# xyyandhtl/IsaacgymLoco

Measured on AMD Instinct MI355X. Metric: env-steps/sec (whole node), higher is better.
Workload: dtype f32; 1 GPU; aliengo: HIMOnPolicyRunner loop, 9 whole PPO iteration(s) timed, each = 100 x (policy inference + LeggedRobot.step + storage) + GAE + HIMPPO.update (5 epochs x 4 minibatches), 4096 envs/GPU; task=aliengo, envs_per_gpu=4096, mode=train, parallelism=dp1, mixed_robots=False, full=False

## Files before the change

### include/lsim.h

```cpp
#ifndef LSIM_H
#define LSIM_H

#include <stddef.h>
#include <stdint.h>

#ifdef __cplusplus
extern "C" {
#endif

#define LSIM_ABI_VERSION 7

#define LSIM_NUM_DOF 12
#define LSIM_NUM_BODIES 17
#define LSIM_NUM_LEGS 4
#define LSIM_NUM_ACTIONS 12
#define LSIM_ONE_STEP_OBS 45
#define LSIM_OBS_HISTORY 6
#define LSIM_NUM_OBS 270
#define LSIM_MAX_HEIGHT_PTS_X 32
#define LSIM_MAX_HEIGHT_PTS_Y 32
#define LSIM_NUM_HEIGHT_PTS 187
#define LSIM_NUM_PRIV_OBS 238
#define LSIM_NUM_AMP_OBS 30
#define LSIM_NUM_BASE_HEIGHT_PTS 63
// ... 374 lines not shown

int lsim_policy_act_at(const lsim_him_policy* p, const lsim_rollout_storage* st, int64_t step_idx, int64_t draw_counter,
                       const float* obs, const float* priv_obs, const float* std, uint32_t seed, uint32_t rank,
                       float* mean_out, float* values_out, float* actions_out, void* stream);

int lsim_policy_act_post_at(const lsim_him_policy* p, const lsim_rollout_storage* st, int64_t step_idx, int64_t draw_counter,
                            const float* obs, const float* priv_obs, const float* std, uint32_t seed, uint32_t rank,
                            float* mean_out, float* values_out, float* actions_out,
                            int64_t prev_step, const uint8_t* prev_dones, const uint8_t* prev_time_outs, const float* prev_rewards,
                            const float* prev_term_priv_obs, float gamma, void* stream);

typedef struct lsim_policy_extra {
    const float* rows;
    int32_t dim, ld;
    float* store;
} lsim_policy_extra;
int lsim_policy_forward_ext(const lsim_him_policy* p, const lsim_policy_extra* extra, const float* obs, const float* priv_obs, int64_t num_envs,
                            float* mean_out, float* values_out, void* stream);
int lsim_policy_act_post_at_ext(const lsim_him_policy* p, const lsim_policy_extra* extra, const lsim_rollout_storage* st, int64_t step_idx,
                                int64_t draw_counter, const float* obs, const float* priv_obs, const float* std, uint32_t seed, uint32_t rank,
                                float* mean_out, float* values_out, float* actions_out,
                                int64_t prev_step, const uint8_t* prev_dones, const uint8_t* prev_time_outs, const float* prev_rewards,
                                const float* prev_term_priv_obs, float gamma, void* stream);

typedef struct lsim_amp_disc {
    lsim_mlp_layer hidden[2];
    const float* head_weight;
    const float* head_bias;
    const double* norm_mean;
    const double* norm_var;
    double norm_eps, norm_clip;
    double reward_coef, task_reward_lerp;
    int32_t amp_dim, reserved;
} lsim_amp_disc;
int lsim_amp_step_workspace(int64_t num_envs, size_t* bytes);
int lsim_amp_step(const lsim_amp_disc* d, const float* amp_obs, const float* next_amp_obs, const uint8_t* dones, const float* terminal_amp_states,
                  const float* task_rewards, int64_t num_envs, float* rewards_out, float* disc_out, float* amp_obs_carry,
                  float* replay_states, float* replay_next_states, int64_t replay_capacity, int64_t replay_cursor,
                  void* workspace, size_t workspace_bytes, void* stream);

int lsim_linear_wgrad_workspace(long batch, int k_in, int n_out, size_t* bytes, int* num_waves);
int lsim_linear_wgrad(const float* x, int64_t ldx, const float* g, int64_t ldg, int64_t batch, int k_in, int n_out,
                      float* dw, float* db, void* workspace, size_t workspace_bytes, void* stream);

int lsim_linear_elu_forward(const float* x, int64_t ldx, const float* weight, const float* bias, int64_t batch, int k_in, int n_out,
                            float* out, int64_t ldo, void* stream);

int lsim_linear_elu_wgrad(const float* x, int64_t ldx, const float* grad_out, int64_t ldg, const float* elu_out, int64_t ldz, int64_t batch,
                          int k_in, int n_out, float* dw, float* db, float* grad_pre, void* workspace, size_t workspace_bytes, void* stream);

int lsim_linear_relu_wgrad(const float* x, int64_t ldx, const float* grad_out, int64_t ldg, const float* relu_out, int64_t ldz, int64_t batch,
                           int k_in, int n_out, float* dw, float* db, float* grad_pre, void* workspace, size_t workspace_bytes, void* stream);

int lsim_linear_masked_forward(const float* x, int64_t ldx, const float* weight, const float* mask_src, int64_t ldm, int64_t batch, int k_in, int n_out,
                               float* out, int64_t ldo, void* stream);

int lsim_relu_cols_workspace(int64_t batch, int n, size_t* bytes);
int lsim_relu_head_backward(const float* relu_out, int64_t ld, const float* grad_d, const float* head_weight, int64_t batch, int n,
                            float* grad_pre, float* grad_bias, float* grad_head, void* workspace, size_t workspace_bytes, void* stream);
int lsim_masked_colsum(const float* v, int64_t ldv, const float* mask_src, int64_t ldm, int64_t batch, int n, float* out,
                       void* workspace, size_t workspace_bytes, void* stream);

int lsim_running_moments_workspace(size_t* bytes);
int lsim_running_moments_update(const float* x, int64_t ldx, int64_t batch, int dim, double* mean, double* var, double* count,
                                void* workspace, size_t workspace_bytes, void* stream);

int lsim_amp_pair_rows(const float* states, int64_t ld_states, const float* next_states, int64_t ld_next, const double* norm_mean,
                       const double* norm_var, double norm_eps, double norm_clip, int64_t batch, int dim, float* out, int64_t ld_out, void* stream);

typedef struct lsim_wgrad_pending {
    const float* part; const float* part2;
    float* out; float* out2;
    int32_t num_partials, count, count2, reserved;
} lsim_wgrad_pending;
int lsim_linear_wgrad_deferred(const float* x, int64_t ldx, const float* g, int64_t ldg, int64_t batch, int k_in, int n_out,
                               float* dw, float* db, void* workspace, size_t workspace_bytes, void* stream, lsim_wgrad_pending* pending);
int lsim_linear_elu_wgrad_deferred(const float* x, int64_t ldx, const float* grad_out, int64_t ldg, const float* elu_out, int64_t ldz, int64_t batch,
                                   int k_in, int n_out, float* dw, float* db, float* grad_pre, void* workspace, size_t workspace_bytes, void* stream,
                                   lsim_wgrad_pending* pending);
int lsim_linear_relu_wgrad_deferred(const float* x, int64_t ldx, const float* grad_out, int64_t ldg, const float* relu_out, int64_t ldz, int64_t batch,
                                    int k_in, int n_out, float* dw, float* db, float* grad_pre, void* workspace, size_t workspace_bytes, void* stream,
                                    lsim_wgrad_pending* pending);
int lsim_wgrad_reduce_batch(const lsim_wgrad_pending* items, int n, void* stream);

int lsim_gather_rows(const void* src, int64_t cols, const int64_t* index, int64_t n, void* dst, void* stream);
int lsim_gather_rows_ld(const void* src, int64_t cols, const int64_t* index, int64_t n, void* dst, int64_t dst_ld, void* stream);

int lsim_normalize_rows(float* w, int rows, int cols, float eps, void* stream);

int lsim_ppo_loss_workspace(long batch, size_t* bytes);
int lsim_ppo_loss(const float* mu, const float* sigma, const float* value, const float* actions, const float* old_logp, const float* advantages,
                  const float* returns, const float* target_values, const float* old_mu, const float* old_sigma, int64_t batch, int num_actions,
                  float clip_param, float value_loss_coef, float entropy_coef, int use_clipped_value_loss,
                  float* out5, float* grad_mu, float* grad_sigma, float* grad_value, void* workspace, size_t workspace_bytes, void* stream);
int lsim_ppo_loss_std_workspace(long batch, int num_actions, size_t* bytes);
int lsim_ppo_loss_std(const float* mu, const float* std, const float* value, const float* actions, const float* old_logp, const float* advantages,
                      const float* returns, const float* target_values, const float* old_mu, const float* old_sigma, int64_t batch, int num_actions,
                      float clip_param, float value_loss_coef, float entropy_coef, int use_clipped_value_loss,
                      float* out5, float* grad_mu, float* grad_std, float* grad_value, void* workspace, size_t workspace_bytes, void* stream);


int lsim_adaptive_lr(const float* kl_mean_dev, float desired_kl, float lr_min, float lr_max, float factor, float* lr_dev, void* stream);

int lsim_sinkhorn_workspace(long batch, int K, size_t* bytes);
int lsim_sinkhorn(const float* scores, int64_t lds, int64_t batch, int K, float eps, int iters, float* out,
                  void* workspace, size_t workspace_bytes, void* stream);

int lsim_estimator_loss_workspace(int64_t batch, int latent, int K, size_t* bytes);
int lsim_estimator_loss(const float* enc_out, int64_t ld_enc, const float* tgt_out, int64_t ld_tgt, const float* proto, const float* vel,
                        int64_t ld_vel, int64_t batch, int latent, int K, float temperature, float sinkhorn_eps, int sinkhorn_iters,
                        float* losses3, float* grad_enc, float* grad_tgt, float* grad_proto, void* workspace, size_t workspace_bytes,
                        void* stream);

int lsim_adam_clip_step_workspace(int count, size_t* bytes);
int lsim_adam_clip_step(int count, const int64_t* numel, float* const* params, float* const* grads, float* const* exp_avg,
                        float* const* exp_avg_sq, float* const* steps, const float* lr_dev, float lr_host, float beta1, float beta2,
                        float eps, float max_grad_norm, float* grad_norm_out, void* workspace, size_t workspace_bytes, void* stream);

int lsim_adam_clip_step_ex(int count, const int64_t* numel, float* const* params, float* const* grads, float* const* exp_avg,
                           float* const* exp_avg_sq, float* const* steps, const float* weight_decay, int clip_count,
                           const float* lr_dev, float lr_host, float beta1, float beta2, float eps, float max_grad_norm,
                           float* grad_norm_out, void* workspace, size_t workspace_bytes, void* stream);

int lsim_actor_input(const float* obs, int64_t ld_obs, int num_one_step_obs, const float* enc_out, int64_t ld_enc, int latent,
                     int64_t batch, float* out, void* stream);

#define LSIM_EVAL_BY_ROBOT 1u
#define LSIM_EVAL_BY_TYPE 2u
#define LSIM_EVAL_BY_LEVEL 4u
#define LSIM_EVAL_MAX_GROUPS 4096
#define LSIM_EVAL_MAX_TRACE_ENVS 64
#define LSIM_EVAL_SAT_PERMILLE 980
enum lsim_eval_word {
    LSIM_EVAL_W_SAMPLES = 0,
    LSIM_EVAL_W_LIN_ERR,
    LSIM_EVAL_W_LIN_ERR_SQ,
    LSIM_EVAL_W_YAW_ERR,
    LSIM_EVAL_W_YAW_ERR_SQ,
    LSIM_EVAL_W_POWER,
    LSIM_EVAL_W_TORQUE_SQ,
    LSIM_EVAL_W_ACTION_RATE,
    LSIM_EVAL_W_FEET_CONTACT,
    LSIM_EVAL_W_TORQUE_SAT,
    LSIM_EVAL_W_PEAK_TORQUE_RATIO,
    LSIM_EVAL_W_EPISODES,
    LSIM_EVAL_W_TIME_OUTS,
    LSIM_EVAL_W_FALLS,
    LSIM_EVAL_W_RETURN,
    LSIM_EVAL_W_LENGTH,
    LSIM_EVAL_W_DISTANCE,
    LSIM_EVAL_W_NONFINITE,
    LSIM_EVAL_WORDS
};
#define LSIM_EVAL_TR_DOF_POS_TARGET 0
#define LSIM_EVAL_TR_DOF_POS 12
#define LSIM_EVAL_TR_DOF_VEL 24
#define LSIM_EVAL_TR_TORQUES 36
#define LSIM_EVAL_TR_COMMANDS 48
#define LSIM_EVAL_TR_BASE_LIN_VEL 51
#define LSIM_EVAL_TR_BASE_ANG_VEL 54
#define LSIM_EVAL_TR_CONTACT_FORCES_Z 57
#define LSIM_EVAL_TR_ROOT_POS 61
#define LSIM_EVAL_TR_ROOT_QUAT 64
#define LSIM_EVAL_TR_REW 68
#define LSIM_EVAL_TR_RESET 69
#define LSIM_EVAL_TRACE_DIM 70
// ... 431 lines not shown
```

### isaacgymloco_amd/csrc/ls_learn.h

```cpp
#pragma once
#include <hip/hip_runtime.h>

typedef float ls_v4f __attribute__((ext_vector_type(4)));

#define LS_WGRAD_WAVES_PER_BLOCK 4

template <int NT, int KT>
__global__ __launch_bounds__(64 * LS_WGRAD_WAVES_PER_BLOCK) void lsim_k_linear_wgrad(const float* __restrict__ x, long ldx, const float* __restrict__ g, long ldg,
                                                                                    long batch, int k_in, int n_out, long rows_per_wave,
                                                                                    float* __restrict__ part_dw, float* __restrict__ part_db) {
    const int lane = threadIdx.x & 63, wave = blockIdx.x * LS_WGRAD_WAVES_PER_BLOCK + (threadIdx.x >> 6);
    const int sub = lane >> 4, col = lane & 15;
    const long b0 = (long)wave * rows_per_wave;
    if (b0 >= batch) return;
    long b1 = b0 + rows_per_wave;
    if (b1 > batch) b1 = batch;
    ls_v4f acc[NT][KT];
    float dbacc[NT];
#pragma unroll
    for (int nt = 0; nt < NT; ++nt) {
        dbacc[nt] = 0.0f;
#pragma unroll
        for (int kt = 0; kt < KT; ++kt) acc[nt][kt] = (ls_v4f){0.0f, 0.0f, 0.0f, 0.0f};
    }
// ... 518 lines not shown
        }
        if (bad) return LSIM_E_UNSUPPORTED;
    } else {
        const int tiles = p.n_blocks * p.k_blocks;
        const int blocks = tiles * p.partials;
        const int vx = ((ldx % 4 == 0) && (((uintptr_t)x & 15) == 0)) ? 2 : (((ldx % 2 == 0) && (((uintptr_t)x & 7) == 0)) ? 1 : 0);
        int vg = ((ldg % 4 == 0) && (((uintptr_t)g & 15) == 0)) ? 2 : 0;
        if (fz && !((ldz % 4 == 0) && (((uintptr_t)z & 15) == 0))) vg = 0;
        const int kg = k_in <= 64 ? 1 : 2;
#define LS_T(VX, VG, KG, FZ) hipLaunchKernelGGL((lsim_k_linear_wgrad_tiled<VX, VG, KG, FZ>), dim3(blocks), dim3(256), 0, s, x, (long)ldx, g, (long)ldg, z, (long)ldz, \
                                                gy, (long)batch, k_in, n_out, p.k_blocks, tiles, p.partials, p.rows, pdw, pdb, zoff)
#define LS_TZ(VX, VG, KG) do { if (fz) LS_T(VX, VG, KG, true); else LS_T(VX, VG, KG, false); } while (0)
#define LS_TK(VX, VG) do { if (kg == 1) LS_TZ(VX, VG, 1); else LS_TZ(VX, VG, 2); } while (0)
        if (vg == 2) { if (vx == 2) LS_TK(2, 2); else if (vx == 1) LS_TK(1, 2); else LS_TK(0, 2); }
        else         { if (vx == 2) LS_TK(2, 0); else if (vx == 1) LS_TK(1, 0); else LS_TK(0, 0); }
#undef LS_TK
#undef LS_TZ
#undef LS_T
    }
    const int count = n_out * k_in;
    if (pending) {
        pending->part = pdw; pending->part2 = pdb; pending->out = dw; pending->out2 = db;
        pending->num_partials = p.partials; pending->count = count; pending->count2 = db ? n_out : 0; pending->reserved = 0;
        return hipGetLastError() == hipSuccess ? LSIM_OK : LSIM_E_HIP;
    }
    hipLaunchKernelGGL(lsim_k_wgrad_reduce, dim3(ls_reduce_blocks(pdw, count) + (db ? (n_out + 15) / 16 : 0)), dim3(256), 0, s, (const float*)pdw, p.partials, count, dw,
                       (const float*)pdb, n_out, db);
    return hipGetLastError() == hipSuccess ? LSIM_OK : LSIM_E_HIP;
}

extern "C" int lsim_linear_wgrad_deferred(const float* x, int64_t ldx, const float* g, int64_t ldg, int64_t batch, int k_in, int n_out,
                                          float* dw, float* db, void* workspace, size_t workspace_bytes, void* stream, lsim_wgrad_pending* pending) {
    if (!pending) return LSIM_E_INVALID;
    return ls_linear_wgrad_impl(x, ldx, g, ldg, nullptr, 0, nullptr, batch, k_in, n_out, dw, db, workspace, workspace_bytes, stream, pending);
}
extern "C" int lsim_linear_elu_wgrad_deferred(const float* x, int64_t ldx, const float* grad_out, int64_t ldg, const float* elu_out, int64_t ldz, int64_t batch,
                                              int k_in, int n_out, float* dw, float* db, float* grad_pre, void* workspace, size_t workspace_bytes, void* stream,
                                              lsim_wgrad_pending* pending) {
    if (!elu_out || !pending) return LSIM_E_INVALID;
    return ls_linear_wgrad_impl(x, ldx, grad_out, ldg, elu_out, ldz, grad_pre, batch, k_in, n_out, dw, db, workspace, workspace_bytes, stream, pending);
}
extern "C" int lsim_wgrad_reduce_batch(const lsim_wgrad_pending* items, int n, void* stream) {
    if (n < 0 || (n > 0 && !items)) return LSIM_E_INVALID;
    for (int i0 = 0; i0 < n; i0 += LS_REDUCE_BATCH) {
        LsReduceBatch b;
        b.n = n - i0 < LS_REDUCE_BATCH ? n - i0 : LS_REDUCE_BATCH;
        int blocks = 0;
        for (int i = 0; i < b.n; ++i) {
            const lsim_wgrad_pending& p = items[i0 + i];
            if (!p.part || !p.out || p.num_partials <= 0 || p.count <= 0 || (p.count2 > 0 && (!p.part2 || !p.out2))) return LSIM_E_INVALID;
            b.it[i] = p;
            b.first[i] = blocks;
            blocks += ls_reduce_blocks(p.part, p.count) + (p.count2 > 0 ? (p.count2 + 15) / 16 : 0);
        }
        b.first[b.n] = blocks;
        hipLaunchKernelGGL(lsim_k_wgrad_reduce_batch, dim3(blocks), dim3(256), 0, (hipStream_t)stream, b);
    }
    return hipGetLastError() == hipSuccess ? LSIM_OK : LSIM_E_HIP;
}

extern "C" int lsim_linear_wgrad(const float* x, int64_t ldx, const float* g, int64_t ldg, int64_t batch, int k_in, int n_out,
                                 float* dw, float* db, void* workspace, size_t workspace_bytes, void* stream) {
    return ls_linear_wgrad_impl(x, ldx, g, ldg, nullptr, 0, nullptr, batch, k_in, n_out, dw, db, workspace, workspace_bytes, stream);
}

extern "C" int lsim_linear_elu_wgrad(const float* x, int64_t ldx, const float* grad_out, int64_t ldg, const float* elu_out, int64_t ldz, int64_t batch,
                                     int k_in, int n_out, float* dw, float* db, float* grad_pre, void* workspace, size_t workspace_bytes, void* stream) {
    if (!elu_out) return LSIM_E_INVALID;
    return ls_linear_wgrad_impl(x, ldx, grad_out, ldg, elu_out, ldz, grad_pre, batch, k_in, n_out, dw, db, workspace, workspace_bytes, stream);
}

extern "C" int lsim_linear_relu_wgrad(const float* x, int64_t ldx, const float* grad_out, int64_t ldg, const float* relu_out, int64_t ldz, int64_t batch,
                                      int k_in, int n_out, float* dw, float* db, float* grad_pre, void* workspace, size_t workspace_bytes, void* stream) {
    if (!relu_out) return LSIM_E_INVALID;
    return ls_linear_wgrad_impl(x, ldx, grad_out, ldg, relu_out, ldz, grad_pre, batch, k_in, n_out, dw, db, workspace, workspace_bytes, stream, nullptr, 0.0f);
}
extern "C" int lsim_linear_relu_wgrad_deferred(const float* x, int64_t ldx, const float* grad_out, int64_t ldg, const float* relu_out, int64_t ldz, int64_t batch,
                                               int k_in, int n_out, float* dw, float* db, float* grad_pre, void* workspace, size_t workspace_bytes, void* stream,
                                               lsim_wgrad_pending* pending) {
    if (!relu_out || !pending) return LSIM_E_INVALID;
    return ls_linear_wgrad_impl(x, ldx, grad_out, ldg, relu_out, ldz, grad_pre, batch, k_in, n_out, dw, db, workspace, workspace_bytes, stream, pending, 0.0f);
}

#define LS_SK_ROWS 256

template <int KMAX>
__device__ __forceinline__ void ls_row_load(const float* __restrict__ p, int K, bool vec, float fill, float (&v)[KMAX]) {
    if (vec) {
#pragma unroll
        for (int k = 0; k < KMAX; k += 4) {
            const float4 t = *(const float4*)(p + (k < K ? k : 0));
            v[k] = k < K ? t.x : fill; v[k + 1] = k < K ? t.y : fill; v[k + 2] = k < K ? t.z : fill; v[k + 3] = k < K ? t.w : fill;
        }
    } else {
#pragma unroll
        for (int k = 0; k < KMAX; ++k) { const float t = p[k < K ? k : 0]; v[k] = k < K ? t : fill; }
    }
}
template <int KMAX>
__device__ __forceinline__ void ls_row_store(float* __restrict__ p, int K, bool vec, const float (&v)[KMAX]) {
    if (vec) {
#pragma unroll
        for (int k = 0; k < KMAX; k += 4) if (k < K) *(float4*)(p + k) = make_float4(v[k], v[k + 1], v[k + 2], v[k + 3]);
    } else {
#pragma unroll
        for (int k = 0; k < KMAX; ++k) if (k < K) p[k] = v[k];
    }
}

#define LS_COLSUM_TILE(KMAX) (128 * ((KMAX) + 1))
template <int KMAX>
__device__ __forceinline__ void ls_block_colsum(const float (&v)[KMAX], float* __restrict__ tile, float* __restrict__ part_row , int K) {
    constexpr int G = 256 / KMAX;
    const int t = threadIdx.x, k = t & (KMAX - 1), g = t / KMAX;
    float s = 0.0f;
    for (int round = 0; round < 2; ++round) {
        __syncthreads();
        if ((t >> 7) == round) {
#pragma unroll
            for (int j = 0; j < KMAX; ++j) tile[(t & 127) * (KMAX + 1) + j] = v[j];
        }
        __syncthreads();
        for (int r = g; r < 128; r += G) s += tile[r * (KMAX + 1) + k];
    }
    __syncthreads();
    tile[g * (KMAX + 1) + k] = s;
    __syncthreads();
    if (t < K) {
        float a = 0.0f;
#pragma unroll
        for (int j = 0; j < G; ++j) a += tile[j * (KMAX + 1) + t];
        part_row[t] = a;
    }
}

template <int KMAX>
__global__ __launch_bounds__(256) void lsim_k_sinkhorn_first(const float* __restrict__ scores, long lds, long scores_mat_stride, long batch, int K,
                                                             float inv_eps, bool vec_in, float* __restrict__ E, float* __restrict__ part) {
    __shared__ float tile[LS_COLSUM_TILE(KMAX)];
    const long m = blockIdx.y, b = (long)blockIdx.x * LS_SK_ROWS + threadIdx.x;
    const bool vec = (K & 3) == 0;
    float v[KMAX];
#pragma unroll
    for (int k = 0; k < KMAX; ++k) v[k] = 0.0f;
    if (b < batch) {
        ls_row_load<KMAX>(scores + m * scores_mat_stride + b * lds, K, vec_in, 0.0f, v);
#pragma unroll
        for (int k = 0; k < KMAX; ++k) v[k] = k < K ? expf(v[k] * inv_eps) : 0.0f;
        ls_row_store<KMAX>(E + (m * batch + b) * K, K, vec, v);
    }
    ls_block_colsum<KMAX>(v, tile, part + (m * gridDim.x + blockIdx.x) * K, K);
}

template <int KMAX>
__global__ __launch_bounds__(256) void lsim_k_sinkhorn_mid(const float* __restrict__ E, const float* __restrict__ u, long batch, int K,
                                                           float* __restrict__ part) {
    __shared__ float tile[LS_COLSUM_TILE(KMAX)];
    __shared__ float us[KMAX];
    const long m = blockIdx.y, b = (long)blockIdx.x * LS_SK_ROWS + threadIdx.x;
    if (threadIdx.x < KMAX) us[threadIdx.x] = (int)threadIdx.x < K ? u[m * 64 + threadIdx.x] : 0.0f;
    __syncthreads();
    float v[KMAX];
#pragma unroll
    for (int k = 0; k < KMAX; ++k) v[k] = 0.0f;
    if (b < batch) {
        ls_row_load<KMAX>(E + (m * batch + b) * K, K, (K & 3) == 0, 0.0f, v);
// ... 943 lines not shown
```

### isaacgymloco_amd/learn/fused_linear.py

```python
import ctypes
import os
import weakref

import torch
import torch.nn as nn
import torch.nn.functional as F

_MIN_BATCH = 4096
_workspaces = {}
_plans = {}
_adam_tables = {}


def _workspace(kind, device, nbytes, floor=0):
    key = (kind, device, torch.cuda.current_stream(device).cuda_stream)
    ws = _workspaces.get(key)
    if ws is None or ws.numel() < nbytes:
        ws = torch.empty(max(int(nbytes), int(floor)), dtype=torch.uint8, device=device)
        _workspaces[key] = ws
    return ws


class GradArena:

# ... 167 lines not shown
    act = () if kind == "none" else (act_out.data_ptr(), act_out.stride(0))
    args = ((x.data_ptr(), x.stride(0), g.data_ptr(), g.stride(0)) + act + (batch, k_in, n_out, dw.data_ptr(), ptr(db))
            + (() if kind == "none" else (ptr(grad_pre),)) + (ws.data_ptr(), ws.numel(), torch.cuda.current_stream(x.device).cuda_stream))
    fn = "lsim_linear_wgrad" if kind == "none" else f"lsim_linear_{kind}_wgrad"
    lib.check(_wgrad_call(L, fn, fn + "_deferred", args, weight_ptr, ws, (x, g) if kind == "none" else (x, g, act_out),
                          arena and (hit[0] or _defer_without_arena)), what=fn)
    return dw, db, grad_pre


def linear_wgrad(x, g, want_bias=True, weight_ptr=None, bias_ptr=None):
    if x.stride(1) != 1:
        x = x.contiguous()
    if g.stride(1) != 1:
        g = g.contiguous()
    return _wgrad_launch("none", x, g, None, weight_ptr, bias_ptr, want_bias)[:2]


class _SkinnyLinearFn(torch.autograd.Function):
    @staticmethod
    def forward(ctx, x, weight, bias):
        ctx.save_for_backward(x, weight)
        ctx.has_bias = bias is not None
        ctx.bias_ptr = bias.data_ptr() if bias is not None else None
        return F.linear(x, weight, bias)

    @staticmethod
    def backward(ctx, g):
        x, weight = ctx.saved_tensors
        gx = g @ weight if ctx.needs_input_grad[0] else None
        dw = db = None
        if ctx.needs_input_grad[1] or (ctx.has_bias and ctx.needs_input_grad[2]):
            dw, db = linear_wgrad(x, g, want_bias=ctx.has_bias, weight_ptr=weight.data_ptr(), bias_ptr=ctx.bias_ptr)
        return gx, dw, db


def _eligible_fused_elu(batch, k_in, n_out):
    return _eligible(batch, k_in, n_out) and k_in * n_out > 4096


def _fused_forward_wanted(x, k_in):
    mode = os.environ.get("LSIM_ELU_FORWARD", "aligned")
    if mode == "aligned":
        return x.stride(0) % 4 == 0 and x.data_ptr() % 16 == 0 and k_in % 4 == 0
    return mode != "0"


def linear_elu_forward(x, weight, bias):
    if (x.is_cuda and x.dim() == 2 and x.dtype == torch.float32 and weight.dtype == torch.float32 and weight.is_contiguous() and weight.shape[0] % 4 == 0
            and x.shape[1] == weight.shape[1] and (bias is None or (bias.dtype == torch.float32 and bias.is_contiguous() and bias.numel() == weight.shape[0]))
            and x.stride(1) == 1 and _fused_forward_wanted(x, weight.shape[1])):
        from .. import abi, lib
        z = torch.empty(x.shape[0], weight.shape[0], device=x.device, dtype=torch.float32)
        b = bias.detach() if bias is not None else None
        rc = lib.load().lsim_linear_elu_forward(x.data_ptr(), x.stride(0), weight.data_ptr(), b.data_ptr() if b is not None else None, x.shape[0],
                                                weight.shape[1], weight.shape[0], z.data_ptr(), z.stride(0), torch.cuda.current_stream(x.device).cuda_stream)
        if rc == 0:
            return z
        if rc != abi.E_UNSUPPORTED:
            lib.check(rc, what="lsim_linear_elu_forward")
    return F.elu(F.linear(x, weight, bias))


class _LinearEluFn(torch.autograd.Function):

    @staticmethod
    def forward(ctx, x, weight, bias):
        z = linear_elu_forward(x, weight, bias)
        ctx.save_for_backward(x, weight, z)
        ctx.has_bias = bias is not None
        ctx.bias_ptr = bias.data_ptr() if bias is not None else None
        return z

    @staticmethod
    def backward(ctx, g):
        x, weight, z = ctx.saved_tensors
        if x.stride(1) != 1:
            x = x.contiguous()
        dw, db, g_pre = _wgrad_launch("elu", x, g.contiguous(), z, weight.data_ptr(), ctx.bias_ptr, want_bias=ctx.has_bias,
                                      want_grad_pre=ctx.needs_input_grad[0])
        gx = g_pre @ weight if g_pre is not None else None
        return gx, dw, db


class HimMLP(nn.Sequential):

    def forward(self, x):
        mods = list(self)
        i = 0
        fuse = x.is_cuda and x.dim() == 2 and x.dtype == torch.float32 and torch.is_grad_enabled()
        while i < len(mods):
            m = mods[i]
            nxt = mods[i + 1] if i + 1 < len(mods) else None
            if (fuse and isinstance(m, nn.Linear) and m.weight.requires_grad and isinstance(nxt, nn.ELU) and nxt.alpha == 1.0 and not nxt.inplace
                    and _eligible_fused_elu(x.shape[0], m.in_features, m.out_features)):
                x = _LinearEluFn.apply(x, m.weight, m.bias)
                i += 2
            else:
                x = m(x)
                i += 1
        return x


class SkinnyLinear(nn.Linear):
    def forward(self, x):
        if (x.is_cuda and x.dim() == 2 and x.dtype == torch.float32 and torch.is_grad_enabled() and self.weight.requires_grad
                and _eligible(x.shape[0], self.in_features, self.out_features)):
            return _SkinnyLinearFn.apply(x, self.weight, self.bias)
        return F.linear(x, self.weight, self.bias)


def sinkhorn_hip(scores, eps, iters):
    from .. import lib
    L = lib.load()
    if scores.stride(1) != 1:
        scores = scores.contiguous()
    B, K = scores.shape
    need = ctypes.c_size_t()
    lib.check(L.lsim_sinkhorn_workspace(B, K, ctypes.byref(need)), what="lsim_sinkhorn_workspace")
    ws = _workspace("sinkhorn", scores.device, need.value)
    out = torch.empty(B, K, device=scores.device, dtype=torch.float32)
    lib.check(L.lsim_sinkhorn(scores.data_ptr(), scores.stride(0), B, K, float(eps), int(iters), out.data_ptr(), ws.data_ptr(), ws.numel(),
                              torch.cuda.current_stream(scores.device).cuda_stream), what="lsim_sinkhorn")
    return out


class _PpoLossFn(torch.autograd.Function):

    @staticmethod
    def forward(ctx, mu, sigma, value, actions, old_logp, adv, returns, target_values, old_mu, old_sigma, clip, vcoef, ecoef, clipped, out=None):
        from .. import lib
        L = lib.load()
        c = lambda t: t.detach().contiguous()
        mu_, sg_, v_ = c(mu), c(sigma), c(value).reshape(-1)
        B, A = mu_.shape
        std_mode = sg_.dim() == 1
        need = ctypes.c_size_t()
        if std_mode:
            lib.check(L.lsim_ppo_loss_std_workspace(B, A, ctypes.byref(need)), what="lsim_ppo_loss_std_workspace")
        else:
            lib.check(L.lsim_ppo_loss_workspace(B, ctypes.byref(need)), what="lsim_ppo_loss_workspace")
        ws = torch.empty(need.value, dtype=torch.uint8, device=mu.device)
        if out is None:
            out = torch.empty(5, device=mu.device)
        g_mu, g_sg, g_v = torch.empty_like(mu_), torch.empty_like(sg_), torch.empty_like(v_)
        args = [c(t).reshape(B, -1) if t is not None else None for t in (actions, old_logp, adv, returns, target_values, old_mu, old_sigma)]
        ptr = lambda t: t.data_ptr() if t is not None else None
        fn = L.lsim_ppo_loss_std if std_mode else L.lsim_ppo_loss
        lib.check(fn(mu_.data_ptr(), sg_.data_ptr(), v_.data_ptr(), ptr(args[0]), ptr(args[1]), ptr(args[2]), ptr(args[3]), ptr(args[4]),
                     ptr(args[5]), ptr(args[6]), B, A, float(clip), float(vcoef), float(ecoef), int(bool(clipped)), out.data_ptr(),
                     g_mu.data_ptr(), g_sg.data_ptr(), g_v.data_ptr(), ws.data_ptr(), ws.numel(),
                     torch.cuda.current_stream(mu.device).cuda_stream), what="lsim_ppo_loss")
        ctx.save_for_backward(g_mu, g_sg, g_v)
        ctx.value_shape = value.shape
        _PpoLossFn.last_grads = (g_mu, g_sg, g_v.reshape(value.shape))
        stats = out[:4]
        ctx.mark_non_differentiable(stats)
        return out[4], stats

    @staticmethod
    def backward(ctx, g_loss, _g_stats):
        g_mu, g_sg, g_v = ctx.saved_tensors
        return (g_loss * g_mu, g_loss * g_sg, (g_loss * g_v).reshape(ctx.value_shape)) + (None,) * 12


def ppo_loss_hip(mu, sigma, value, actions, old_logp, adv, returns, target_values, old_mu, old_sigma, clip, vcoef, ecoef, clipped, out=None):
    loss, stats = _PpoLossFn.apply(mu, sigma, value, actions, old_logp, adv, returns, target_values, old_mu, old_sigma, clip, vcoef, ecoef, clipped, out)
    loss._lsim_direct = ((mu, sigma, value), _PpoLossFn.last_grads)
    _PpoLossFn.last_grads = None
    return loss, stats


class _EstimatorLossFn(torch.autograd.Function):

    @staticmethod
    def forward(ctx, enc_out, tgt_out, proto, vel, temperature, eps, iters):
        from .. import lib
        L = lib.load()
# ... 105 lines not shown
```

Measured before the change: 4.965 million env-steps/s.

## Fuse final Linear-ELU-Linear head backward into one MFMA kernel

Adds a HIP kernel that, for the last Linear layer of an MLP preceded by Linear+ELU, computes the head weight/bias gradients and the ELU-masked input gradient in a single pass. It uses MFMA with the head weight staged in LDS. HimMLP now detects the trailing Linear-ELU-Linear pattern and routes it through a new autograd function. This replaces a separate wgrad launch, a dgrad GEMM and the ELU backward. The aim is to cut kernel launches and memory traffic for the small-output heads during PPO update, at the cost of more per-block LDS and register use plus another reduction over partials.

Result: no change. 4.994 million env-steps/s, median of 6 (+0.6%).

```diff
diff --git a/include/lsim.h b/include/lsim.h
--- a/include/lsim.h
+++ b/include/lsim.h
@@ -480,6 +480,13 @@
                                     int k_in, int n_out, float* dw, float* db, float* grad_pre, void* workspace, size_t workspace_bytes, void* stream,
                                     lsim_wgrad_pending* pending);
 int lsim_wgrad_reduce_batch(const lsim_wgrad_pending* items, int n, void* stream);
+
+int lsim_linear_head_elu_backward_workspace(int64_t batch, int k_in, int n_out, size_t* bytes, int* num_partials);
+int lsim_linear_head_elu_backward(const float* elu_out, int64_t ldz, const float* g, int64_t ldg, const float* weight, int64_t batch, int k_in,
+                                  int n_out, float* grad_pre, float* dw, float* db, void* workspace, size_t workspace_bytes, void* stream);
+int lsim_linear_head_elu_backward_deferred(const float* elu_out, int64_t ldz, const float* g, int64_t ldg, const float* weight, int64_t batch,
+                                           int k_in, int n_out, float* grad_pre, float* dw, float* db, void* workspace, size_t workspace_bytes,
+                                           void* stream, lsim_wgrad_pending* pending);
 
 int lsim_gather_rows(const void* src, int64_t cols, const int64_t* index, int64_t n, void* dst, void* stream);
 int lsim_gather_rows_ld(const void* src, int64_t cols, const int64_t* index, int64_t n, void* dst, int64_t dst_ld, void* stream);
diff --git a/isaacgymloco_amd/csrc/ls_learn.h b/isaacgymloco_amd/csrc/ls_learn.h
--- a/isaacgymloco_amd/csrc/ls_learn.h
+++ b/isaacgymloco_amd/csrc/ls_learn.h
@@ -624,6 +624,237 @@
     return ls_linear_wgrad_impl(x, ldx, grad_out, ldg, relu_out, ldz, grad_pre, batch, k_in, n_out, dw, db, workspace, workspace_bytes, stream, pending, 0.0f);
 }
 
+#define LS_HEAD_BLOCKS 512
+#define LS_HEAD_MAX_N 32
+#define LS_HEAD_MAX_K 128
+
+template <bool VEC> __device__ __forceinline__ float4 ls_head_ld4(const float* __restrict__ p) {
+    if (VEC) return *(const float4*)p;
+    return make_float4(p[0], p[1], p[2], p[3]);
+}
+
+template <int NT, int KQ, bool VEC>
+__global__ __launch_bounds__(64 * LS_WGRAD_WAVES_PER_BLOCK) void lsim_k_head_elu_backward(const float* __restrict__ z, long ldz, const float* __restrict__ g, long ldg,
+                                                                                         const float* __restrict__ W, long batch, int k_in, int n_out,
+                                                                                         long rows_per_block, float* __restrict__ grad_pre,
+                                                                                         float* __restrict__ part_dw, float* __restrict__ part_db) {
+    constexpr int WS = KQ * 64 + 16;
+    constexpr int NS = NT * 4;
+    constexpr int NRED = NT * KQ * 16 + NT;
+    constexpr int LDS_W = NT * 16 * WS, LDS_R = 3 * NRED * 64;
+    __shared__ float lds[LDS_W > LDS_R ? LDS_W : LDS_R];
+    float* Ws = lds;
+    for (int i = threadIdx.x; i < NT * 16 * WS; i += 64 * LS_WGRAD_WAVES_PER_BLOCK) {
+        const int n = i / WS, j = i - n * WS;
+        Ws[i] = (n < n_out && j < k_in) ? W[(long)n * k_in + j] : 0.0f;
+    }
+    __syncthreads();
+    const int lane = threadIdx.x & 63, wave = threadIdx.x >> 6;
+    const int sub = lane >> 4, col = lane & 15;
+    const long b0 = (long)blockIdx.x * rows_per_block;
+    long b1 = b0 + rows_per_block;
+    if (b1 > batch) b1 = batch;
+    const int ns = (n_out + 3) >> 2, jt_n = (k_in + 15) >> 4;
+    ls_v4f acc[NT][KQ][4];
+    float dbacc[NT];
+    int gn[NT], zc[KQ];
+#pragma unroll
+    for (int nt = 0; nt < NT; ++nt) {
+        dbacc[nt] = 0.0f;
+        const int n = nt * 16 + col;
+        gn[nt] = n < n_out ? n : n_out - 1;
+#pragma unroll
+        for (int q = 0; q < KQ; ++q)
+#pragma unroll
+            for (int r = 0; r < 4; ++r) acc[nt][q][r] = (ls_v4f){0.0f, 0.0f, 0.0f, 0.0f};
+    }
+#pragma unroll
+    for (int q = 0; q < KQ; ++q) { const int c = q * 64 + 4 * col; zc[q] = c < k_in ? c : k_in - 4; }
+    for (long b = b0 + 16 * wave; b < b1; b += 16 * LS_WGRAD_WAVES_PER_BLOCK) {
+        float a[4][NT];
+        float4 zz[4][KQ];
+#pragma unroll
+        for (int s = 0; s < 4; ++s) {
+            const long row = b + 4 * s + sub;
+            const bool ok = row < b1;
+            const long r_ = ok ? row : b0;
+#pragma unroll
+            for (int nt = 0; nt < NT; ++nt) { const float t = g[r_ * ldg + gn[nt]]; a[s][nt] = ok ? t : 0.0f; }
+#pragma unroll
+            for (int q = 0; q < KQ; ++q) {
+                const float4 t = ls_head_ld4<VEC>(z + r_ * ldz + zc[q]);
+                zz[s][q] = ok ? t : make_float4(0.0f, 0.0f, 0.0f, 0.0f);
+            }
+        }
+        const long rowc = b + col;
+        const bool okc = rowc < b1;
+        const long rc = okc ? rowc : b0;
+        float gb[NS];
+#pragma unroll
+        for (int st = 0; st < NS; ++st) {
+            const int n = 4 * st + sub;
+            gb[st] = 0.0f;
+            if (st < ns) { const float t = g[rc * ldg + (n < n_out ? n : n_out - 1)]; gb[st] = (okc && n < n_out) ? t : 0.0f; }
+        }
+        float4 zb[4 * KQ];
+#pragma unroll
+        for (int t = 0; t < 4 * KQ; ++t) {
+            const int c = t * 16 + 4 * sub;
+            zb[t] = make_float4(0.0f, 0.0f, 0.0f, 0.0f);
+            if (t < jt_n) zb[t] = ls_head_ld4<VEC>(z + rc * ldz + (c < k_in ? c : k_in - 4));
+        }
+#pragma unroll
+        for (int s = 0; s < 4; ++s)
+#pragma unroll
+            for (int nt = 0; nt < NT; ++nt) {
+                dbacc[nt] += a[s][nt];
+#pragma unroll
+                for (int q = 0; q < KQ; ++q) {
+                    acc[nt][q][0] = __builtin_amdgcn_mfma_f32_16x16x4f32(a[s][nt], zz[s][q].x, acc[nt][q][0], 0, 0, 0);
+                    acc[nt][q][1] = __builtin_amdgcn_mfma_f32_16x16x4f32(a[s][nt], zz[s][q].y, acc[nt][q][1], 0, 0, 0);
+                    acc[nt][q][2] = __builtin_amdgcn_mfma_f32_16x16x4f32(a[s][nt], zz[s][q].z, acc[nt][q][2], 0, 0, 0);
+                    acc[nt][q][3] = __builtin_amdgcn_mfma_f32_16x16x4f32(a[s][nt], zz[s][q].w, acc[nt][q][3], 0, 0, 0);
+                }
+            }
+#pragma unroll
+        for (int t = 0; t < 4 * KQ; ++t) {
+            if (t >= jt_n) continue;
+            ls_v4f G = (ls_v4f){0.0f, 0.0f, 0.0f, 0.0f};
+#pragma unroll
+            for (int st = 0; st < NS; ++st)
+                if (st < ns) G = __builtin_amdgcn_mfma_f32_16x16x4f32(Ws[(4 * st + sub) * WS + t * 16 + col], gb[st], G, 0, 0, 0);
+            const int c = t * 16 + 4 * sub;
+            if (okc && c < k_in) {
+                const float4 v = zb[t];
+                *(float4*)(grad_pre + rowc * k_in + c) = make_float4(G[0] * (v.x > 0.0f ? 1.0f : v.x + 1.0f), G[1] * (v.y > 0.0f ? 1.0f : v.y + 1.0f),
+                                                                     G[2] * (v.z > 0.0f ? 1.0f : v.z + 1.0f), G[3] * (v.w > 0.0f ? 1.0f : v.w + 1.0f));
+            }
+        }
+    }
+    float dbv[NT];
+#pragma unroll
+    for (int nt = 0; nt < NT; ++nt) {
+        float v = dbacc[nt];
+        v += __shfl_xor(v, 16, 64);
+        v += __shfl_xor(v, 32, 64);
+        dbv[nt] = v;
+    }
+    __syncthreads();
+    if (wave > 0) {
+        float* red = lds + (size_t)(wave - 1) * NRED * 64 + lane;
+#pragma unroll
+        for (int nt = 0; nt < NT; ++nt) {
+#pragma unroll
+            for (int q = 0; q < KQ; ++q)
+#pragma unroll
+                for (int u = 0; u < 4; ++u)
+#pragma unroll
+                    for (int r = 0; r < 4; ++r) red[(((nt * KQ + q) * 4 + u) * 4 + r) * 64] = acc[nt][q][u][r];
+            red[(NT * KQ * 16 + nt) * 64] = dbv[nt];
+        }
+    }
+    __syncthreads();
+    if (wave > 0) return;
+#pragma unroll 1
+    for (int o = 0; o < 3; ++o) {
+        const float* red = lds + (size_t)o * NRED * 64 + lane;
+#pragma unroll
+        for (int nt = 0; nt < NT; ++nt) {
+#pragma unroll
+            for (int q = 0; q < KQ; ++q)
+#pragma unroll
+                for (int u = 0; u < 4; ++u)
+#pragma unroll
+                    for (int r = 0; r < 4; ++r) acc[nt][q][u][r] += red[(((nt * KQ + q) * 4 + u) * 4 + r) * 64];
+            dbv[nt] += red[(NT * KQ * 16 + nt) * 64];
+        }
+    }
+    float* pw = part_dw + (size_t)blockIdx.x * n_out * k_in;
+#pragma unroll
+    for (int nt = 0; nt < NT; ++nt)
+#pragma unroll
+        for (int q = 0; q < KQ; ++q)
+#pragma unroll
+            for (int r = 0; r < 4; ++r) {
+                const int n = nt * 16 + 4 * sub + r, k = q * 64 + 4 * col;
+                if (n < n_out && k < k_in) *(float4*)(pw + (size_t)n * k_in + k) = make_float4(acc[nt][q][0][r], acc[nt][q][1][r], acc[nt][q][2][r], acc[nt][q][3][r]);
+            }
+    if (part_db) {
+#pragma unroll
+        for (int nt = 0; nt < NT; ++nt) {
+            const int n = nt * 16 + col;
+            if (sub == 0 && n < n_out) part_db[(size_t)blockIdx.x * n_out + n] = dbv[nt];
+        }
+    }
+}
+
+struct LsHeadPlan { long rows; int partials; };
+static int ls_head_plan(long batch, int k_in, int n_out, LsHeadPlan* p) {
+    LsWgradPlan w;
+    const int rc = ls_wgrad_plan(batch, k_in, n_out, &w);
+    if (rc != LSIM_OK) return rc;
+    if (!w.small || n_out > LS_HEAD_MAX_N || k_in > LS_HEAD_MAX_K || (k_in & 3) != 0) return LSIM_E_UNSUPPORTED;
+    long rpb = ((batch + LS_HEAD_BLOCKS - 1) / LS_HEAD_BLOCKS + 15) & ~15L;
+    if (rpb < 16) rpb = 16;
+    p->rows = rpb;
+    p->partials = (int)((batch + rpb - 1) / rpb);
+    return LSIM_OK;
+}
+static size_t ls_head_workspace_bytes(const LsHeadPlan& p, int k_in, int n_out) {
+    return (size_t)p.partials * ((size_t)n_out * k_in + n_out) * sizeof(float);
+}
+extern "C" int lsim_linear_head_elu_backward_workspace(int64_t batch, int k_in, int n_out, size_t* bytes, int* num_partials) {
+    if (!bytes || !num_partials) return LSIM_E_INVALID;
+    LsHeadPlan p;
+    const int rc = ls_head_plan(batch, k_in, n_out, &p);
+    if (rc != LSIM_OK) return rc;
+    *num_partials = p.partials;
+    *bytes = ls_head_workspace_bytes(p, k_in, n_out);
+    return LSIM_OK;
+}
+
+static int ls_head_elu_backward_impl(const float* z, int64_t ldz, const float* g, int64_t ldg, const float* W, int64_t batch, int k_in, int n_out,
+                                     float* grad_pre, float* dw, float* db, void* workspace, size_t workspace_bytes, void* stream,
+                                     lsim_wgrad_pending* pending) {
+    if (!z || !g || !W || !grad_pre || !dw || !workspace) return LSIM_E_INVALID;
+    LsHeadPlan p;
+    const int rc = ls_head_plan(batch, k_in, n_out, &p);
+    if (rc != LSIM_OK) return rc;
+    if (ldz < k_in || ldg < n_out || workspace_bytes < ls_head_workspace_bytes(p, k_in, n_out)) return LSIM_E_INVALID;
+    if ((((uintptr_t)grad_pre) & 15) != 0 || (((uintptr_t)workspace) & 15) != 0) return LSIM_E_INVALID;
+    float* pdw = (float*)workspace;
+    float* pdb = db ? pdw + (size_t)p.partials * n_out * k_in : nullptr;
+    hipStream_t s = (hipStream_t)stream;
+    const int blocks = p.partials;
+    const bool vec = (ldz % 4 == 0) && ((((uintptr_t)z) & 15) == 0);
+#define LS_H(NT, KQ, VEC) hipLaunchKernelGGL((lsim_k_head_elu_backward<NT, KQ, VEC>), dim3(blocks), dim3(64 * LS_WGRAD_WAVES_PER_BLOCK), 0, s, z, (long)ldz, g, (long)ldg, \
+                                             W, (long)batch, k_in, n_out, p.rows, grad_pre, pdw, pdb)
+#define LS_HV(NT, KQ) do { if (vec) LS_H(NT, KQ, true); else LS_H(NT, KQ, false); } while (0)
+    if (n_out <= 16) { if (k_in <= 64) LS_HV(1, 1); else LS_HV(1, 2); }
+    else             { if (k_in <= 64) LS_HV(2, 1); else LS_HV(2, 2); }
+#undef LS_HV
+#undef LS_H
+    const int count = n_out * k_in;
+    if (pending) {
+        pending->part = pdw; pending->part2 = pdb; pending->out = dw; pending->out2 = db;
+        pending->num_partials = p.partials; pending->count = count; pending->count2 = db ? n_out : 0; pending->reserved = 0;
+        return hipGetLastError() == hipSuccess ? LSIM_OK : LSIM_E_HIP;
+    }
+    hipLaunchKernelGGL(lsim_k_wgrad_reduce, dim3(ls_reduce_blocks(pdw, count) + (db ? (n_out + 15) / 16 : 0)), dim3(256), 0, s, (const float*)pdw, p.partials, count, dw,
+                       (const float*)pdb, n_out, db);
+    return hipGetLastError() == hipSuccess ? LSIM_OK : LSIM_E_HIP;
+}
+extern "C" int lsim_linear_head_elu_backward(const float* elu_out, int64_t ldz, const float* g, int64_t ldg, const float* weight, int64_t batch, int k_in,
+                                             int n_out, float* grad_pre, float* dw, float* db, void* workspace, size_t workspace_bytes, void* stream) {
+    return ls_head_elu_backward_impl(elu_out, ldz, g, ldg, weight, batch, k_in, n_out, grad_pre, dw, db, workspace, workspace_bytes, stream, nullptr);
+}
+extern "C" int lsim_linear_head_elu_backward_deferred(const float* elu_out, int64_t ldz, const float* g, int64_t ldg, const float* weight, int64_t batch,
+                                                      int k_in, int n_out, float* grad_pre, float* dw, float* db, void* workspace, size_t workspace_bytes,
+                                                      void* stream, lsim_wgrad_pending* pending) {
+    if (!pending) return LSIM_E_INVALID;
+    return ls_head_elu_backward_impl(elu_out, ldz, g, ldg, weight, batch, k_in, n_out, grad_pre, dw, db, workspace, workspace_bytes, stream, pending);
+}
+
 #define LS_SK_ROWS 256
 
 template <int KMAX>
diff --git a/isaacgymloco_amd/learn/fused_linear.py b/isaacgymloco_amd/learn/fused_linear.py
--- a/isaacgymloco_amd/learn/fused_linear.py
+++ b/isaacgymloco_amd/learn/fused_linear.py
@@ -273,6 +273,66 @@
         return gx, dw, db
 
 
+_head_plans = {}
+
+
+def _eligible_head(batch, k_in, n_out):
+    if batch < _MIN_BATCH or os.environ.get("LSIM_HEAD_BACKWARD", "1") == "0":
+        return False
+    key = (batch, k_in, n_out)
+    ok = _head_plans.get(key)
+    if ok is None:
+        from .. import lib
+        need, parts = ctypes.c_size_t(), ctypes.c_int()
+        ok = lib.load().lsim_linear_head_elu_backward_workspace(batch, k_in, n_out, ctypes.byref(need), ctypes.byref(parts)) == 0
+        _head_plans[key] = ok
+    return ok
+
+
+def _head_backward_launch(z, g, weight, bias_ptr, want_bias=True):
+    from .. import lib
+    L = lib.load()
+    batch, k_in = z.shape
+    n_out = g.shape[1]
+    need, parts = ctypes.c_size_t(), ctypes.c_int()
+    lib.check(L.lsim_linear_head_elu_backward_workspace(batch, k_in, n_out, ctypes.byref(need), ctypes.byref(parts)), what="lsim_linear_head_elu_backward_workspace")
+    weight_ptr = weight.data_ptr()
+    per_param = _pending is not None
+    ws = _workspace(("head", weight_ptr) if per_param else "head", z.device, need.value, floor=0 if per_param else 1 << 20)
+    hit = [True]
+    dw = _grad_out(weight_ptr, (n_out, k_in), z.device, hit)
+    db = _grad_out(bias_ptr, (n_out,), z.device, hit) if want_bias else None
+    grad_pre = torch.empty(batch, k_in, device=z.device, dtype=torch.float32)
+    args = (z.data_ptr(), z.stride(0), g.data_ptr(), g.stride(0), weight_ptr, batch, k_in, n_out, grad_pre.data_ptr(), dw.data_ptr(),
+            db.data_ptr() if db is not None else None, ws.data_ptr(), ws.numel(), torch.cuda.current_stream(z.device).cuda_stream)
+    fn = "lsim_linear_head_elu_backward"
+    lib.check(_wgrad_call(L, fn, fn + "_deferred", args, weight_ptr, ws, (z, g, weight), hit[0] or _defer_without_arena), what=fn)
+    return grad_pre, dw, db
+
+
+class _LinearEluHeadFn(torch.autograd.Function):
+
+    @staticmethod
+    def forward(ctx, x, w1, b1, w2, b2):
+        z = linear_elu_forward(x, w1, b1)
+        ctx.save_for_backward(x, w1, z, w2)
+        ctx.b1_ptr = b1.data_ptr() if b1 is not None else None
+        ctx.b2_ptr = b2.data_ptr() if b2 is not None else None
+        return F.linear(z, w2, b2)
+
+    @staticmethod
+    def backward(ctx, g):
+        x, w1, z, w2 = ctx.saved_tensors
+        if x.stride(1) != 1:
+            x = x.contiguous()
+        if g.stride(1) != 1:
+            g = g.contiguous()
+        grad_pre, dw2, db2 = _head_backward_launch(z, g, w2.detach(), ctx.b2_ptr, want_bias=ctx.b2_ptr is not None)
+        dw1, db1, _ = _wgrad_launch("none", x, grad_pre, None, w1.data_ptr(), ctx.b1_ptr, want_bias=ctx.b1_ptr is not None)
+        gx = grad_pre @ w1 if ctx.needs_input_grad[0] else None
+        return gx, dw1, db1, dw2, db2
+
+
 class HimMLP(nn.Sequential):
 
     def forward(self, x):
@@ -282,8 +342,15 @@
         while i < len(mods):
             m = mods[i]
             nxt = mods[i + 1] if i + 1 < len(mods) else None
-            if (fuse and isinstance(m, nn.Linear) and m.weight.requires_grad and isinstance(nxt, nn.ELU) and nxt.alpha == 1.0 and not nxt.inplace
-                    and _eligible_fused_elu(x.shape[0], m.in_features, m.out_features)):
+            head = mods[i + 2] if i + 3 == len(mods) else None
+            pair = (fuse and isinstance(m, nn.Linear) and m.weight.requires_grad and isinstance(nxt, nn.ELU) and nxt.alpha == 1.0 and not nxt.inplace
+                    and _eligible_fused_elu(x.shape[0], m.in_features, m.out_features))
+            if (pair and isinstance(head, nn.Linear) and head.weight.requires_grad and head.weight.is_contiguous() and head.weight.dtype == torch.float32
+                    and head.in_features == m.out_features and (m.bias is None or m.bias.requires_grad) and (head.bias is None or head.bias.requires_grad)
+                    and _eligible_head(x.shape[0], head.in_features, head.out_features)):
+                x = _LinearEluHeadFn.apply(x, m.weight, m.bias, head.weight, head.bias)
+                i += 3
+            elif pair:
                 x = _LinearEluFn.apply(x, m.weight, m.bias)
                 i += 2
             else:
```
